# RIKEN-RCCS/EigenExa

Hardware: AMD Instinct MI355X
Metric: eigen_sx full-solve throughput (reference flop model: 4/3 N^3 + D&C GEMM + 2 nvec N^2) (higher is better)
Workload: dtype f64; 1 GPU; N=8192 random symmetric fp64 (counter-based R+R^T, seed 20240807), eigen_sx all eigenpairs, m_forward=64, m_backward=128; parallelism=1 GPU (1x1 grid)

## Files before the change

eigenexa_amd/_lib.py:

```python
import ctypes as C
import os

_HERE = os.path.dirname(os.path.abspath(__file__))
LIB_PATH = os.environ.get("EIGX_LIB") or os.path.join(_HERE, "lib", "libeigenexa_amd.so")

_c_double_p = C.POINTER(C.c_double)
_c_int_p = C.POINTER(C.c_int)

_INT, _PTR = C.c_int, C.c_void_p
_SOLVE = [_INT, _INT, _PTR, _INT, _PTR, _PTR, _INT, _INT, _INT, C.c_char]
_SOLVE_BC = [_INT, _INT, _INT, _PTR, _INT, _PTR, _PTR, _INT, _INT, _INT, _INT, C.c_char]
_RANGE = [_INT, _INT, _INT, _PTR, _INT, _PTR, _PTR, _INT, _INT, _INT, C.c_char]
_RANGE_V = [_INT, C.c_double, C.c_double, _INT, _c_int_p, _c_int_p, _PTR, _INT, _PTR, _PTR, _INT, _INT, _INT, C.c_char]
_GEV = [_INT, _PTR, _INT, _PTR, _INT, _PTR, _PTR, _INT]
_GEV_RANGE = [_INT, _INT, _INT, _PTR, _INT, _PTR, _INT, _PTR, _PTR, _INT, C.c_char]
_GEV_RANGE_V = [_INT, C.c_double, C.c_double, _INT, _c_int_p, _c_int_p, _PTR, _INT, _PTR, _INT, _PTR, _PTR, _INT, C.c_char]
_BATCH = [_INT, _INT, _PTR, _INT, C.c_int64, _PTR, _INT, _PTR, _INT, C.c_int64, C.c_char, _PTR]
_GEV_BATCH = [_INT, _INT, _PTR, _INT, C.c_int64, _PTR, _INT, C.c_int64, _PTR, _INT, _PTR, _INT, C.c_int64, C.c_char, _PTR]
_INDEX = [_INT, _INT, _INT]
_CHOL = [_INT, _PTR, _INT]
_TRSM = [C.c_char, _INT, _INT, _PTR, _INT, _PTR, _INT]
_REDUCE = [_INT, _PTR, _INT, _PTR, _INT]

SIGNATURES = {
# ... 132 lines not shown
}

HBATCH_RANGE_SIGNATURES = {
    "eigx_h_batch_range": (C.c_int, _BATCH_RANGE),
    "eigx_h_batch_range_dev": (C.c_int, _BATCH_RANGE),
}

LAB_SIGNATURES = {
    "eigx_dgemm_ex_dev": (C.c_int, [C.c_char, C.c_char, _INT, _INT, _INT, C.c_double, _PTR, _INT, _PTR, _INT, C.c_double, _PTR,
                                    _INT, _INT, _INT, _INT, _INT, _INT, _INT, C.c_int64, C.c_int64, C.c_int64, _INT, C.c_int64,
                                    C.c_int64, C.c_int64, _INT, _INT, _PTR, _PTR]),
    "eigx_dgemm_tri2_launch_tiles": (C.c_int, [_INT] * 8),
    "eigx_dgemm_gather_table_dev": (C.c_int, [_INT, _PTR, _PTR, _INT, _PTR, _INT, _PTR, _INT, _PTR, _PTR]),
}

_lib = None


def load():
    global _lib
    if _lib is not None:
        return _lib
    if not os.path.exists(LIB_PATH):
        raise RuntimeError(
            f"{LIB_PATH} not found: build it with tools/build_lib.sh (hipcc --offload-arch=gfx950). "
            "eigenexa_amd has no CPU fallback."
        )
    lib = C.CDLL(LIB_PATH, mode=C.RTLD_GLOBAL)
    for name, (res, args) in {**SIGNATURES, **GBATCH_SIGNATURES, **HGBATCH_SIGNATURES, **VBATCH_SIGNATURES,
                               **GVBATCH_SIGNATURES, **BATCH_RANGE_SIGNATURES, **HBATCH_RANGE_SIGNATURES}.items():
        fn = getattr(lib, name)
        fn.restype = res
        fn.argtypes = args
    for name, (res, args) in LAB_SIGNATURES.items():
        fn = getattr(lib, name, None)
        if fn is not None:
            fn.restype = res
            fn.argtypes = args
    _lib = lib
    return lib


def check(rc, what):
    if rc != 0:
        raise RuntimeError(f"{what} failed with code {rc}")
```

eigenexa_amd/csrc/api.hip:

```cpp
#include "eigx_context.h"
#include "eigx_comm.h"
#include "../../include/eigenexa_amd.h"
#include <cstring>

namespace eigx {
Context g_ctx;
}

using namespace eigx;

extern "C" {

int eigx_init(int device) {
  return eigx_init_multi(device, 0, 1, nullptr, 'C');
}

int eigx_get_device_count(void) {
  int ndev = 0;
  if (hipGetDeviceCount(&ndev) != hipSuccess) { (void)hipGetLastError(); return 0; }
  return ndev;
}

int eigx_get_rccl_unique_id(void* out128) {
  return comm_get_unique_id(out128);
// ... 313 lines not shown
  if (key == 6) return set_gemm_cstream(value);
  if (key == 7) return value > 0 ? set_reduce_knob(key, value) : -1;
  if (key == 8) return set_dc_chunk(value);
  if (key == 9) return comm_set_bounce(value);
  if (key == 15) return set_dc_pipe(value);
  if (key == 16) return set_dc_batch(value);
  if (key == 17 || key == 18 || key == 19) return set_range_knob(key, value);
  if (key == 20) return set_tri_nb(value);
  if (key == 21) return set_batch_nmax(value);
  if (key == 22) return set_hbatch_nmax(value);
  if (key == 23) return set_gbatch_nmax(value);
  if (key == 24) return set_hgbatch_nmax(value);
  if (key == 25) return set_gemm_latec_kmax(value);
  if (key == 26) return set_batch_range_route(value);
  if (key == 27) return set_batch_range_accept(value);
  return -1;
}

int eigx_dgemm_dev(char opa, char opb, int m, int n, int k, double alpha, const double* a, int lda,
                   const double* b, int ldb, double beta, double* c, int ldc, int tri_upper) {
  if (!g_ctx.initialized) return EIGX_ERR_NOT_INITIALIZED;
  EIGX_HIP_CHECK(hipStreamSynchronize(nullptr));
  dgemm_dev(g_ctx.stream, opa, opb, m, n, k, alpha, a, lda, b, ldb, beta, c, ldc, tri_upper ? 1 : 0,
            &g_ctx.grid);
  EIGX_HIP_CHECK(hipStreamSynchronize(g_ctx.stream));
  return EIGX_OK;
}

int eigx_dgemm_gather_dev(char opa, char opb, int m, int n, int k, double alpha, const double* a, int lda,
                          const double* b, int ldb, double beta, double* c, int ldc, const int* kmap_a,
// ... 11 lines not shown
```

eigenexa_amd/csrc/eigx_common.h:

```cpp
#pragma once
#include <hip/hip_runtime.h>
#include <cstdio>
#include <cstdlib>
#include <cstdint>
#include <cmath>
#include <vector>
#include <ctime>
#include <chrono>

#define EIGX_HIP_CHECK(expr)                                                        \
  do {                                                                              \
    hipError_t _e = (expr);                                                         \
    if (_e != hipSuccess) {                                                         \
      fprintf(stderr, "[eigx] HIP error %s at %s:%d: %s\n", hipGetErrorName(_e),    \
              __FILE__, __LINE__, hipGetErrorString(_e));                           \
      abort();                                                                      \
    }                                                                               \
  } while (0)

namespace eigx {

typedef double d4_t __attribute__((ext_vector_type(4)));

struct Grid {
// ... 42 lines not shown
};
inline char upper_case(char c) { return (c >= 'a' && c <= 'z') ? (char)(c - 'a' + 'A') : c; }
inline SolveRequest normalize_request(int n, int nvec, char mode) {
  mode = upper_case(mode);
  if (nvec == 0) mode = 'N';
  if (nvec < 0) nvec = -nvec;
  if (nvec > n) nvec = n;
  return SolveRequest{mode, nvec, mode != 'N'};
}


__global__ void fill_kernel(double* p, size_t n, double v);
__global__ void fill_vec_kernel(double* __restrict__ w, int n, double v);
__global__ void scale_vec_kernel(double* __restrict__ w, int n, double s);

void dgemm_dev(hipStream_t stream, char opA, char opB, int M, int N, int K, double alpha,
               const double* A, int lda, const double* B, int ldb, double beta, double* C, int ldc,
               int tri_mode = 0, const Grid* g = nullptr, const int* kmapA = nullptr,
               const int* cmapC = nullptr, int batch = 1, long strideA = 0, long strideB = 0, long strideC = 0,
               int batch2 = 1, long strideA2 = 0, long strideB2 = 0, long strideC2 = 0, int ownP = 1,
               int ownp = 0, const int* kmapB = nullptr, int tn_lo = 0, int tn_hi = 0x7fffffff);

int gemm_tri2_launch_tiles(int M, int N, const Grid& g, int tn_lo, int tn_hi);

struct GemmBatch {
  int M, N, K, pad;
  long offA, offB, offC;
  int offKA, offKB;
};
void dgemm_gather_batch_dev(hipStream_t stream, const GemmBatch* tab_dev, int nbatch, int maxM, int maxN,
                            const double* A, int lda, const double* B, int ldb, double* C, int ldc,
                            const int* kmapA, const int* kmapB);

inline void stage_trace(int rank, const char* what, long detail = -1) {
  static const bool on = getenv("EIGX_TRACE_STAGES") != nullptr;
  if (!on) return;
  timespec ts;
  clock_gettime(CLOCK_MONOTONIC, &ts);
  if (detail >= 0) fprintf(stderr, "[eigx stage] rank %d t=%.3f %s %ld\n", rank, ts.tv_sec % 100000 + ts.tv_nsec * 1e-9, what, detail);
  else fprintf(stderr, "[eigx stage] rank %d t=%.3f %s\n", rank, ts.tv_sec % 100000 + ts.tv_nsec * 1e-9, what);
  fflush(stderr);
}

int set_gemm_variant(int v);
int set_gemm_cstream(int v);
int set_gemm_latec_kmax(int v);
int set_bisect_threads(int v);
int set_bt_q(int v);
int set_reduce_knob(int key, int v);
int set_dc_chunk(int v);
int set_dc_pipe(int v);
int set_dc_batch(int v);
int set_batch_nmax(int v);
int set_hbatch_nmax(int v);
int get_batch_nmax();
int get_hbatch_nmax();
int set_gbatch_nmax(int v);
int set_hgbatch_nmax(int v);
int get_gbatch_nmax();
int set_batch_range_route(int v);
int set_batch_range_accept(int v);
int get_batch_range_route();
int get_batch_range_accept();
// ... 4 lines not shown
```

eigenexa_amd/csrc/gemm_f64.hip:

```cpp
#include "eigx_common.h"

namespace eigx {

namespace {

constexpr int BK = 16;
constexpr int LD_KC = BK + 1;
template <int WT> struct Geo {
  static constexpr int BM = 2 * WT, BN = 2 * WT;
  static constexpr int LD_MC = BM + 16;
  static constexpr int OPER = (BK * LD_MC > BM * LD_KC) ? BK * LD_MC : BM * LD_KC;
  static constexpr int NL = BM * BK / 256;
  static constexpr int NF = WT / 16;
};

struct GemmArgs {
  int M, N, K;
  double alpha, beta;
  const double* A;
  int lda;
  const double* B;
  int ldb;
  double* C;
  int ldc;
  int tri_mode;
  int Px, px, Py, py;
  const int* kmapA;
  const int* cmapC;
  const int* kmapB;
  long sA, sB, sC;
  long sA2, sB2, sC2;
  int ownP, ownp;
  int tri_gb;
  int tn_lo, tn_hi;
  int c_stream;
  int nrg, rg_h, rg_c1;
  unsigned rg_magic;
  const GemmBatch* btab;
};
__host__ __device__ inline int tri2_c0(const GemmArgs& g, int q, int tiles_n) {
  const long grow_min = (long)q * g.rg_h * 128 * g.Px + g.px;
  const unsigned x = grow_min > g.py ? (unsigned)(grow_min - g.py + g.Py - 1) : 0u;
#ifdef __HIP_DEVICE_COMPILE__
  const unsigned lc = (g.Py == 1) ? x : __umulhi(x, g.rg_magic);
#else
  const unsigned lc = (g.Py == 1) ? x : (unsigned)(((unsigned long long)x * g.rg_magic) >> 32);
#endif
  int c = (lc > (unsigned)(g.N - 1)) ? tiles_n : (int)(lc >> 7);
  if (c < g.tn_lo) c = g.tn_lo;
  if (c > g.rg_c1) c = g.rg_c1;
  return c;
}
typedef double d2s_t __attribute__((ext_vector_type(2)));

template <int WT>
__device__ __forceinline__ void load_map(int (&kc)[Geo<WT>::NL], const int* __restrict__ kmap, int k0, int Kmax,
                                         int tid) {
  constexpr int BM = Geo<WT>::BM, NL = Geo<WT>::NL;
  const int kb = k0 + tid / BM;
#pragma unroll
  for (int p = 0; p < NL; ++p) {
    const int k = kb + (256 / BM) * p;
    kc[p] = kmap[k < Kmax ? k : 0];
  }
}

template <bool KC, int WT, bool MAP>
__device__ __forceinline__ void load_slab(double (&r)[Geo<WT>::NL], const double* __restrict__ P, int ld, int m0,
                                          int k0, int Mmax, int Kmax, int tid, const int (&kc)[Geo<WT>::NL]) {
  constexpr int BM = Geo<WT>::BM, NL = Geo<WT>::NL;
  if (!KC) {
    const int m = m0 + (tid & (BM - 1));
    const int kb = k0 + tid / BM;
    const bool mok = m < Mmax;
    if (MAP) {
#pragma unroll
      for (int p = 0; p < NL; ++p) {
        const int k = kb + (256 / BM) * p;
        r[p] = (mok && k < Kmax) ? P[(size_t)m + (size_t)kc[p] * ld] : 0.0;
      }
    } else {
#pragma unroll
      for (int p = 0; p < NL; ++p) {
        const int k = kb + (256 / BM) * p;
        r[p] = (mok && k < Kmax) ? P[(size_t)m + (size_t)k * ld] : 0.0;
      }
    }
  } else {
    const int k = k0 + (tid & 15);
    const int mb = m0 + (tid >> 4);
    const bool kok = k < Kmax;
#pragma unroll
    for (int p = 0; p < NL; ++p) {
      const int m = mb + 16 * p;
      r[p] = (kok && m < Mmax) ? P[(size_t)k + (size_t)m * ld] : 0.0;
    }
  }
}

template <bool KC, int WT>
__device__ __forceinline__ void store_slab(const double (&r)[Geo<WT>::NL], double* __restrict__ S, int tid) {
  constexpr int BM = Geo<WT>::BM, NL = Geo<WT>::NL, LD_MC = Geo<WT>::LD_MC;
  if (!KC) {
    const int m = tid & (BM - 1);
    const int kb = tid / BM;
#pragma unroll
    for (int p = 0; p < NL; ++p) S[(kb + (256 / BM) * p) * LD_MC + m] = r[p];
  } else {
    const int k = tid & 15;
    const int mb = tid >> 4;
#pragma unroll
    for (int p = 0; p < NL; ++p) S[(mb + 16 * p) * LD_KC + k] = r[p];
  }
}

template <bool KC, int WT>
__device__ __forceinline__ double frag(const double* __restrict__ S, int m, int k) {
  return KC ? S[m * LD_KC + k] : S[k * Geo<WT>::LD_MC + m];
}

template <bool A_KC, bool B_KC, int WT, bool GATHER>
__global__ __launch_bounds__(256, 2) void gemm_f64_kernel(GemmArgs g) {
  extern __shared__ __attribute__((aligned(16))) double smem[];
  constexpr int BM = Geo<WT>::BM, BN = Geo<WT>::BN, OPER_DOUBLES = Geo<WT>::OPER, NL = Geo<WT>::NL, NF = Geo<WT>::NF;
  g.A += (long)blockIdx.y * g.sA + (long)blockIdx.z * g.sA2;
  g.B += (long)blockIdx.y * g.sB + (long)blockIdx.z * g.sB2;
  g.C += (long)blockIdx.y * g.sC + (long)blockIdx.z * g.sC2;
  if (g.btab) {
    const GemmBatch b = g.btab[blockIdx.y];
    g.M = b.M; g.N = b.N; g.K = b.K;
    g.A += b.offA; g.B += b.offB; g.C += b.offC;
    if (GATHER) { g.kmapA += b.offKA; g.kmapB += b.offKB; }
    if ((int)blockIdx.x >= ((g.M + BM - 1) / BM) * ((g.N + BN - 1) / BN)) return;
  }

  const int tid = threadIdx.x;
  const int lane = tid & 63;
// ... 42 lines not shown
          const int m = m0 + wm * WT + i * 16 + fm;
          acc[i][j][r] = (n < g.N && m < g.M) ? cscale * cp[m] : 0.0;
        }
      }
  } else {
#pragma unroll
    for (int j = 0; j < NF; ++j)
#pragma unroll
      for (int i = 0; i < NF; ++i) acc[i][j] = (d4_t){0.0, 0.0, 0.0, 0.0};
  }

  double ra[NL], rb[NL];
  int kca[NL], kcb[NL];
#pragma unroll
  for (int p = 0; p < NL; ++p) { kca[p] = 0; kcb[p] = 0; }
  const int nk = (g.K + BK - 1) / BK;
  if (GATHER) { load_map<WT>(kca, g.kmapA, 0, g.K, tid); load_map<WT>(kcb, g.kmapB, 0, g.K, tid); }
  load_slab<A_KC, WT, GATHER>(ra, g.A, g.lda, m0, 0, g.M, g.K, tid, kca);
  load_slab<B_KC, WT, GATHER>(rb, g.B, g.ldb, n0, 0, g.N, g.K, tid, kcb);
  if (GATHER && nk > 1) { load_map<WT>(kca, g.kmapA, BK, g.K, tid); load_map<WT>(kcb, g.kmapB, BK, g.K, tid); }
  store_slab<A_KC, WT>(ra, smem, tid);
  store_slab<B_KC, WT>(rb, smem + OPER_DOUBLES, tid);
  __syncthreads();

  for (int kt = 0; kt < nk; ++kt) {
    const int cur = kt & 1;
    if (kt + 1 < nk) {
      load_slab<A_KC, WT, GATHER>(ra, g.A, g.lda, m0, (kt + 1) * BK, g.M, g.K, tid, kca);
      load_slab<B_KC, WT, GATHER>(rb, g.B, g.ldb, n0, (kt + 1) * BK, g.N, g.K, tid, kcb);
      if (GATHER && kt + 2 < nk) {
        load_map<WT>(kca, g.kmapA, (kt + 2) * BK, g.K, tid);
        load_map<WT>(kcb, g.kmapB, (kt + 2) * BK, g.K, tid);
      }
    }
    const double* as = smem + cur * 2 * OPER_DOUBLES;
    const double* bs = as + OPER_DOUBLES;
#pragma unroll
    for (int ks = 0; ks < BK / 4; ++ks) {
      double fa[NF], fb[NF];
#pragma unroll
      for (int i = 0; i < NF; ++i) fa[i] = frag<A_KC, WT>(as, wm * WT + i * 16 + fm, ks * 4 + fk);
#pragma unroll
      for (int j = 0; j < NF; ++j) fb[j] = frag<B_KC, WT>(bs, wn * WT + j * 16 + fm, ks * 4 + fk);
#pragma unroll
// ... 75 lines not shown
  asm volatile("s_load_dword %0, %1, %2" : "=s"(v) : "s"(p), "s"(idx * 4) : "memory");
  return v;
}
template <bool MAP>
__device__ __forceinline__ void g2_cols(const int* __restrict__ kmap, int k0, int K, int wave, int& c0, int& c1) {
  const int k = k0 + 2 * wave;
  if (MAP) {
    c0 = 0; c1 = 0;
    if (k < K) c0 = g2_sload(kmap, k);
    if (k + 1 < K) c1 = g2_sload(kmap, k + 1);
  } else {
    c0 = k; c1 = k + 1;
  }
}

template <bool A_KC, bool B_KC, bool GATHER, bool LATE_C = false>
__global__ __launch_bounds__(256, 2) void gemm2_kernel(GemmArgs g) {
  static_assert(!LATE_C || (!A_KC && !B_KC && !GATHER), "late C: plain 'N','T' operands only");
  extern __shared__ __attribute__((aligned(16))) double smem[];
  constexpr int S = 4;
  constexpr int GI = 4;
  constexpr int CI = 8;
  g.A += (long)blockIdx.y * g.sA + (long)blockIdx.z * g.sA2;
  g.B += (long)blockIdx.y * g.sB + (long)blockIdx.z * g.sB2;
  g.C += (long)blockIdx.y * g.sC + (long)blockIdx.z * g.sC2;

  const int tid = threadIdx.x;
  const int lane = tid & 63;
  const int wave = __builtin_amdgcn_readfirstlane(tid >> 6);
  const int wm = wave & 1, wn = wave >> 1;

  const int tiles_m = (g.M + 127) / 128;
  const int tiles_n = (g.N + 127) / 128;
// ... 43 lines not shown
    const int rows = (tiles_m - rg * 8 < 8) ? tiles_m - rg * 8 : 8;
    tn = rem / rows;
    tm = rg * 8 + rem - tn * rows;
  }
  const int m0 = tm * 128, n0 = tn * 128;
  if (g.tri_mode != 0) {
    if (g.ownP > 1 && (tn % g.ownP) != g.ownp) return;
    if (tn < g.tn_lo || tn >= g.tn_hi) return;
    const long grow_min = (long)m0 * g.Px + g.px;
    const int jmax = (n0 + 127 < g.N - 1) ? n0 + 127 : g.N - 1;
    const long gcol_max = (long)jmax * g.Py + g.py;
    if (grow_min > gcol_max) return;
  }

  const int fm = lane & 15, fk = lane >> 4;
  const int nk = (g.K + G2_BK - 1) / G2_BK;

  auto ncol = [&](int j, int rho) { return B_KC ? j * 16 + rho : (j >> 1) * 32 + 2 * rho + (j & 1); };

  d4_t acc[4][4];
  const bool use_c = !LATE_C && (g.beta != 0.0) && (g.alpha != 0.0);
  if (use_c) {
    const double cscale = g.beta / g.alpha;
#pragma unroll
    for (int j = 0; j < 4; ++j)
#pragma unroll
      for (int r = 0; r < 4; ++r) {
        const int n = n0 + wn * 64 + ncol(j, fk + 4 * r);
        const double* cp = g.C + (size_t)n * g.ldc;
        if (!A_KC) {
// ... 245 lines not shown
  g.Px = grid.Px; g.px = grid.px; g.Py = grid.Py; g.py = grid.py;
  return tri2_plan(g);
}

int set_gemm_variant(int v) { const int old = g_gemm_variant; g_gemm_variant = v; return old; }
int set_gemm_cstream(int v) { const int old = g_gemm_cstream; g_gemm_cstream = v; return old; }
int set_gemm_latec_kmax(int v) {
  if (v < 0 || v >= 512) return -1;
  const int old = g_gemm_latec_kmax; g_gemm_latec_kmax = v; return old;
}

void dgemm_dev(hipStream_t stream, char opA, char opB, int M, int N, int K, double alpha, const double* A,
               int lda, const double* B, int ldb, double beta, double* C, int ldc, int tri_mode,
               const Grid* grid, const int* kmapA, const int* cmapC, int batch, long strideA, long strideB,
               long strideC, int batch2, long strideA2, long strideB2, long strideC2, int ownP, int ownp,
               const int* kmapB, int tn_lo, int tn_hi) {
  if (M <= 0 || N <= 0 || batch <= 0 || batch2 <= 0) return;
  if (alpha == 0.0) K = 0;
  GemmArgs g;
  g.M = M; g.N = N; g.K = K; g.alpha = alpha; g.beta = beta;
  g.A = A; g.lda = lda; g.B = B; g.ldb = ldb; g.C = C; g.ldc = ldc;
  g.tri_mode = tri_mode;
  g.kmapA = (opA == 'N' || opA == 'n') ? kmapA : nullptr;
  g.cmapC = cmapC;
  g.kmapB = (opB == 'T' || opB == 't') ? kmapB : nullptr;
  g.sA = strideA; g.sB = strideB; g.sC = strideC;
  g.sA2 = strideA2; g.sB2 = strideB2; g.sC2 = strideC2;
  g.ownP = ownP; g.ownp = ownp; g.tri_gb = 1;
  g.tn_lo = tn_lo; g.tn_hi = tn_hi;
  g.nrg = 0; g.rg_h = 8; g.rg_c1 = 0; g.rg_magic = 0; g.btab = nullptr;
  g.c_stream = (tri_mode != 0 && g_gemm_cstream) ? 1 : 0;
  g.Px = grid ? grid->Px : 1; g.px = grid ? grid->px : 0;
  g.Py = grid ? grid->Py : 1; g.py = grid ? grid->py : 0;
  const bool a_kc = (opA == 'T' || opA == 't');
  const bool b_kc = (opB == 'N' || opB == 'n');
  const bool gather = g.kmapA || g.kmapB;
  if ((!gather || (g.kmapA && g.kmapB && !a_kc && !b_kc)) && gemm2_ok(g, a_kc, b_kc, batch, batch2)) {
    const long t128 = (long)ceil_div(M, 128) * ceil_div(N, 128) * batch * batch2;
    if (tri_mode != 0 || t128 >= 192 || g_gemm_variant == 3) {
      int gx2 = ceil_div(M, 128) * ceil_div(N, 128);
      if (tri_mode == 1) {
        const int t = ceil_div(N > M ? N : M, 128);
        g.tri_gb = (t >= 96) ? 8 : (t >= 24 ? 4 : (t >= 8 ? 2 : 1));
        const int nb = ceil_div(t, g.tri_gb);
        const int nblk = nb * (nb + 1) / 2;
        gx2 = 8 * ceil_div(nblk, 8) * g.tri_gb * g.tri_gb;
      }
      if (tri_mode == 2 && batch == 1 && batch2 == 1 && ownP == 1) {
        const int total = tri2_plan(g);
        if (total == 0) return;
        gx2 = total;
      }
      dim3 grd2(gx2, batch, batch2), blk2(256);
      const size_t shmem2 = (size_t)4 * G2_STAGE * sizeof(double);
#define EIGX_LAUNCH2(AK, BK_, GA_, LC_)                                                            \
  do {                                                                                             \
    static bool attr_set2 = false;                                                                 \
    if (!attr_set2) {                                                                              \
      EIGX_HIP_CHECK(hipFuncSetAttribute((const void*)gemm2_kernel<AK, BK_, GA_, LC_>,             \
                                         hipFuncAttributeMaxDynamicSharedMemorySize, (int)shmem2)); \
      attr_set2 = true;                                                                            \
    }                                                                                              \
    hipLaunchKernelGGL((gemm2_kernel<AK, BK_, GA_, LC_>), grd2, blk2, shmem2, stream, g);          \
  } while (0)
      const bool late_c = tri_mode == 1 && beta != 0.0 && K <= g_gemm_latec_kmax && !g.c_stream;
      if (gather) EIGX_LAUNCH2(false, false, true, false);
      else if (a_kc && b_kc) EIGX_LAUNCH2(true, true, false, false);
      else if (a_kc) EIGX_LAUNCH2(true, false, false, false);
      else if (b_kc) EIGX_LAUNCH2(false, true, false, false);
      else if (late_c) EIGX_LAUNCH2(false, false, false, true);
      else EIGX_LAUNCH2(false, false, false, false);
#undef EIGX_LAUNCH2
      EIGX_HIP_CHECK(hipGetLastError());
      return;
    }
  }
  const long tiles128 = (long)ceil_div(M, 128) * ceil_div(N, 128) * batch * batch2;
  const bool small = (tri_mode == 0) && tiles128 < 192;
  const int bm = small ? 64 : 128;
  const int tiles = ceil_div(M, bm) * ceil_div(N, bm);
  dim3 grd(tiles, batch, batch2), blk(256);
#define EIGX_LAUNCH(AK, BK_, WT_, GA_)                                                             \
  do {                                                                                             \
    const size_t shmem = (size_t)4 * Geo<WT_>::OPER * sizeof(double);                              \
    static bool attr_set = false;                                                                  \
    if (!attr_set) {                                                                               \
      EIGX_HIP_CHECK(hipFuncSetAttribute((const void*)gemm_f64_kernel<AK, BK_, WT_, GA_>,          \
                                         hipFuncAttributeMaxDynamicSharedMemorySize, (int)shmem)); \
      attr_set = true;                                                                             \
    }                                                                                              \
    hipLaunchKernelGGL((gemm_f64_kernel<AK, BK_, WT_, GA_>), grd, blk, shmem, stream, g);          \
  } while (0)
#define EIGX_LAUNCH_T(AK, BK_) do { if (small) EIGX_LAUNCH(AK, BK_, 32, false); else EIGX_LAUNCH(AK, BK_, 64, false); } while (0)
  if (g.kmapA || g.kmapB) {
    if (a_kc || b_kc || !g.kmapA || !g.kmapB) {
      fprintf(stderr, "[eigx] dgemm gather needs opA='N', opB='T' and both maps\n");
      abort();
    }
    if (small) EIGX_LAUNCH(false, false, 32, true); else EIGX_LAUNCH(false, false, 64, true);
  } else if (a_kc && b_kc) EIGX_LAUNCH_T(true, true);
  else if (a_kc && !b_kc) EIGX_LAUNCH_T(true, false);
  else if (!a_kc && b_kc) EIGX_LAUNCH_T(false, true);
  else EIGX_LAUNCH_T(false, false);
#undef EIGX_LAUNCH_T
#undef EIGX_LAUNCH
  EIGX_HIP_CHECK(hipGetLastError());
}

void dgemm_gather_batch_dev(hipStream_t stream, const GemmBatch* tab_dev, int nbatch, int maxM, int maxN,
                            const double* A, int lda, const double* B, int ldb, double* C, int ldc,
                            const int* kmapA, const int* kmapB) {
  if (nbatch <= 0 || maxM <= 0 || maxN <= 0) return;
  GemmArgs g;
  g.M = maxM; g.N = maxN; g.K = 0; g.alpha = 1.0; g.beta = 0.0;
  g.A = A; g.lda = lda; g.B = B; g.ldb = ldb; g.C = C; g.ldc = ldc;
  g.tri_mode = 0; g.kmapA = kmapA; g.cmapC = nullptr; g.kmapB = kmapB;
  g.sA = g.sB = g.sC = 0; g.sA2 = g.sB2 = g.sC2 = 0;
  g.ownP = 1; g.ownp = 0; g.tri_gb = 1; g.tn_lo = 0; g.tn_hi = 0x7fffffff;
  g.nrg = 0; g.rg_h = 8; g.rg_c1 = 0; g.rg_magic = 0; g.c_stream = 0;
  g.Px = 1; g.px = 0; g.Py = 1; g.py = 0;
  g.btab = tab_dev;
  constexpr int WT = 32;
  const int tiles = ceil_div(maxM, Geo<WT>::BM) * ceil_div(maxN, Geo<WT>::BN);
  const size_t shmem = (size_t)4 * Geo<WT>::OPER * sizeof(double);
  static bool attr_set = false;
  if (!attr_set) {
    EIGX_HIP_CHECK(hipFuncSetAttribute((const void*)gemm_f64_kernel<false, false, WT, true>,
                                       hipFuncAttributeMaxDynamicSharedMemorySize, (int)shmem));
    attr_set = true;
  }
  hipLaunchKernelGGL((gemm_f64_kernel<false, false, WT, true>), dim3(tiles, nbatch, 1), dim3(256), shmem, stream, g);
  EIGX_HIP_CHECK(hipGetLastError());
}

// ... 2 lines not shown
```

eigenexa_amd/csrc/gemm_lab.hip:

```cpp
#include "eigx_context.h"
#include "../../include/eigenexa_amd.h"
#include "../../include/eigenexa_amd_gemm_lab.h"
#include <climits>

using namespace eigx;

extern "C" {

int eigx_dgemm_ex_dev(char opa, char opb, int m, int n, int k, double alpha, const double* a, int lda, const double* b,
                      int ldb, double beta, double* c, int ldc, int tri_mode, int px_n, int px, int py_n, int py, int batch,
                      int64_t stride_a, int64_t stride_b, int64_t stride_c, int batch2, int64_t stride_a2, int64_t stride_b2,
                      int64_t stride_c2, int tn_lo, int tn_hi, const int* kmap_a, const int* kmap_b) {
  if (!g_ctx.initialized) return EIGX_ERR_NOT_INITIALIZED;
  if (tri_mode < 0 || tri_mode > 2) return EIGX_ERR_BAD_ARG;
  if (px_n < 1 || py_n < 1 || px < 0 || px >= px_n || py < 0 || py >= py_n) return EIGX_ERR_BAD_ARG;
  if (kmap_a || kmap_b) {
    const bool nt = (opa == 'N' || opa == 'n') && (opb == 'T' || opb == 't');
    if (!nt || !kmap_a || !kmap_b) return EIGX_ERR_BAD_ARG;
  }
  Grid grid;
  grid.Px = px_n; grid.px = px; grid.Py = py_n; grid.py = py;
  grid.nranks = px_n * py_n;
  EIGX_HIP_CHECK(hipStreamSynchronize(nullptr));
  dgemm_dev(g_ctx.stream, opa, opb, m, n, k, alpha, a, lda, b, ldb, beta, c, ldc, tri_mode, &grid, kmap_a, nullptr, batch,
            (long)stride_a, (long)stride_b, (long)stride_c, batch2, (long)stride_a2, (long)stride_b2, (long)stride_c2, 1, 0,
            kmap_b, tn_lo, tn_hi);
  EIGX_HIP_CHECK(hipStreamSynchronize(g_ctx.stream));
  return EIGX_OK;
}

int eigx_dgemm_tri2_launch_tiles(int m, int n, int px_n, int px, int py_n, int py, int tn_lo, int tn_hi) {
  if (px_n < 1 || py_n < 1 || px < 0 || px >= px_n || py < 0 || py >= py_n) return EIGX_ERR_BAD_ARG;
  Grid grid;
  grid.Px = px_n; grid.px = px; grid.Py = py_n; grid.py = py;
  return gemm_tri2_launch_tiles(m, n, grid, tn_lo, tn_hi);
}

int eigx_dgemm_gather_table_dev(int nbatch, const int64_t* entries, const double* a, int lda, const double* b, int ldb,
                                double* c, int ldc, const int* kmap_a, const int* kmap_b) {
  if (!g_ctx.initialized) return EIGX_ERR_NOT_INITIALIZED;
  if (nbatch < 0 || (nbatch > 0 && (!entries || !kmap_a || !kmap_b))) return EIGX_ERR_BAD_ARG;
  if (nbatch == 0) return EIGX_OK;
  std::vector<GemmBatch> tab(nbatch);
// ... 24 lines not shown
```

eigenexa_amd/csrc/trbak.hip:

```cpp
#include "eigx_context.h"
#include "eigx_comm.h"
#include "../../include/eigenexa_amd.h"

namespace eigx {

namespace {

constexpr int GCH = 512;
int g_bt_q = 0;

__global__ void zero_below_kernel(double* __restrict__ A, int lda, int n, int band, int rows_pad) {
  const int j = blockIdx.y;
  const int len = j - band + 1;
  double* col = A + (size_t)j * lda;
  const int lo = len > 0 ? len : 0;
  const int hi = rows_pad < lda ? rows_pad : lda;
  for (int r = lo + blockIdx.x * blockDim.x + threadIdx.x; r < hi; r += gridDim.x * blockDim.x) col[r] = 0.0;
}

__device__ __forceinline__ int tri_idx(int r, int c) { return r * (r + 1) / 2 + c; }

__global__ __launch_bounds__(256) void tbuild_kernel(const double* __restrict__ Gall, int maxchunks, int gch, int mb,
                                                     int mbe, int nsub, int n, const double* __restrict__ A, int lda,
                                                     const double* __restrict__ e, int lde, int band,
// ... 104 lines not shown
  if (q > 1) {
    double* Gs = ctx.pool.get_t<double>("bt.Gs", (size_t)nblk * msz);
    double* Y = ctx.pool.get_t<double>("bt.Y", (size_t)nblk * msz);
    hipLaunchKernelGGL(gsum_kernel, dim3(64, nblk), dim3(256), 0, st, Gall, maxchunks, mbe, Gs);
    for (int h = mb; h < mbe; h *= 2) {
      const int np = mbe / (2 * h);
      const long dstep = (long)2 * h * (mbe + 1);
      dgemm_dev(st, 'N', 'N', h, h, h, 1.0, Gs + h, mbe, Tall, mbe, 0.0, Y, h, 0, nullptr, nullptr, nullptr, np, dstep,
                dstep, (long)h * h, nblk, (long)msz, (long)msz, (long)np * h * h);
      dgemm_dev(st, 'N', 'N', h, h, h, -1.0, Tall + (size_t)h * (mbe + 1), mbe, Y, h, 0.0, Tall + h, mbe, 0, nullptr,
                nullptr, nullptr, np, dstep, (long)h * h, dstep, nblk, (long)msz, (long)np * h * h, (long)msz);
    }
  }
}

static void bt_apply_range(Context& ctx, int nvec, const double* V, int ldv, double* Z, int ldz, int band, int jstart,
                           int jend, int mb, int q) {
  if (jend <= jstart) return;
  hipStream_t st = ctx.stream;
  const BtRange g = bt_range_geom(ctx, band, jstart, jend, mb, q);
  const int mbe = g.mbe;
  double* W = ctx.pool.get_t<double>("bt.W", (size_t)(mbe > 512 ? mbe : 512) * nvec);
  double* X = ctx.pool.get_t<double>("bt.X", (size_t)(mbe > 512 ? mbe : 512) * nvec);
  for (int b = 0; b < g.nblk; ++b) {
    const int j0 = jstart + b * mbe;
    const int mbk = (jend - j0 < mbe) ? jend - j0 : mbe;
    const int rows = j0 + mbk - band;
    const double* Vb = V + (size_t)j0 * ldv;
    const double* T = g.Tall + (size_t)b * g.msz;
    dgemm_dev(st, 'T', 'N', mbk, nvec, rows, 1.0, Vb, ldv, Z, ldz, 0.0, W, mbe);
    dgemm_dev(st, 'N', 'N', mbk, nvec, mbk, 1.0, T, mbe, W, mbe, 0.0, X, mbe);
    dgemm_dev(st, 'N', 'N', rows, nvec, mbk, -1.0, Vb, ldv, X, mbe, 1.0, Z, ldz);
  }
}

struct BtPlan { int mb, q, mbe, js, rows_pad; };
static BtPlan bt_plan(int n, int mb, int band) {
  BtPlan p;
  if (mb < 8) mb = 8;
  if (mb > 128) mb = 128;
  int q = 1;
  if (mb == 128 && n >= 2048) q = (n >= 6144) ? 4 : 2;
  if (g_bt_q > 0 && mb == 128) q = g_bt_q;
  p.mb = mb; p.q = q; p.mbe = mb * q;
  const int total = n - band;
  const int nsup = (q > 1) ? total / p.mbe : 0;
  p.js = (nsup > 0) ? n - nsup * p.mbe : n;
// ... 107 lines not shown
    const BtRange g = bt_range_geom(ctx, band, j0, j1, p.mb, q);
    int rows_pad = g.maxchunks * g.gch;
    if (rows_pad > ldv) rows_pad = ldv;
    hipLaunchKernelGGL(unpack_refl_kernel, dim3(ceil_div(rows_pad, 256) < 64 ? ceil_div(rows_pad, 256) : 64, j1 - j0), dim3(256),
                       0, st, (const double*)recv->local, cnt, nxc, j0, j1, band, rows_pad, G.Px, G.Py, G.row_major, Vg, ldv);
    double* Vs = Vg - (size_t)j0 * ldv;
    bt_prepare_range(ctx, st, n, Vs, ldv, e, lde, band, j0, j1, p.mb, q);
    if (nvec > 0) bt_apply_range(ctx, nvec, Vs, ldv, Z, ldz, band, j0, j1, p.mb, q);
  };
  for (int j0 = band; j0 < p.js; j0 += plain_cols) run_group(j0, (j0 + plain_cols < p.js) ? j0 + plain_cols : p.js, 1);
  for (int j0 = p.js; j0 < n; j0 += group_cols) run_group(j0, (j0 + group_cols < n) ? j0 + group_cols : n, p.q);
  EIGX_HIP_CHECK(hipGetLastError());
}

int set_bt_q(int v) { const int old = g_bt_q; g_bt_q = v; return old; }

}
```

Before: 19470 GFLOP/s.

## Skip structurally zero K ranges in back-transform GEMMs via per-tile K windows

Adds a per-row-tile K window to the f64 GEMM kernels, letting each 128-row tile clamp its reduction range to where the operand is nonzero. The back-transform's three GEMMs pass windows that follow the trapezoidal/triangular shape of the reflector block V and the triangular T, so tiles skip K slabs that are known to be zero. This is meant to cut wasted FLOPs and memory traffic in the Householder back-transformation. The cost is extra kernel template instantiations and a correctness dependence on the assumed zero structure of V and T.

```diff
diff --git a/eigenexa_amd/_lib.py b/eigenexa_amd/_lib.py
--- a/eigenexa_amd/_lib.py
+++ b/eigenexa_amd/_lib.py
@@ -170,6 +170,10 @@
     "eigx_dgemm_gather_table_dev": (C.c_int, [_INT, _PTR, _PTR, _INT, _PTR, _INT, _PTR, _INT, _PTR, _PTR]),
 }
 
+KWIN_LAB_SIGNATURES = {
+    "eigx_dgemm_kwin_dev": (C.c_int, LAB_SIGNATURES["eigx_dgemm_ex_dev"][1] + [_INT, _INT]),
+}
+
 _lib = None
 
 
@@ -188,7 +192,7 @@
         fn = getattr(lib, name)
         fn.restype = res
         fn.argtypes = args
-    for name, (res, args) in LAB_SIGNATURES.items():
+    for name, (res, args) in {**LAB_SIGNATURES, **KWIN_LAB_SIGNATURES}.items():
         fn = getattr(lib, name, None)
         if fn is not None:
             fn.restype = res
diff --git a/eigenexa_amd/csrc/api.hip b/eigenexa_amd/csrc/api.hip
--- a/eigenexa_amd/csrc/api.hip
+++ b/eigenexa_amd/csrc/api.hip
@@ -351,6 +351,7 @@
   if (key == 25) return set_gemm_latec_kmax(value);
   if (key == 26) return set_batch_range_route(value);
   if (key == 27) return set_batch_range_accept(value);
+  if (key == 28) return set_bt_kwin(value);
   return -1;
 }
 
diff --git a/eigenexa_amd/csrc/eigx_common.h b/eigenexa_amd/csrc/eigx_common.h
--- a/eigenexa_amd/csrc/eigx_common.h
+++ b/eigenexa_amd/csrc/eigx_common.h
@@ -3,6 +3,7 @@
 #include <cstdio>
 #include <cstdlib>
 #include <cstdint>
+#include <climits>
 #include <cmath>
 #include <vector>
 #include <ctime>
@@ -80,12 +81,14 @@
 __global__ void fill_vec_kernel(double* __restrict__ w, int n, double v);
 __global__ void scale_vec_kernel(double* __restrict__ w, int n, double s);
 
+constexpr int KWIN_LO_NONE = INT_MIN, KWIN_HI_NONE = INT_MAX;
 void dgemm_dev(hipStream_t stream, char opA, char opB, int M, int N, int K, double alpha,
                const double* A, int lda, const double* B, int ldb, double beta, double* C, int ldc,
                int tri_mode = 0, const Grid* g = nullptr, const int* kmapA = nullptr,
                const int* cmapC = nullptr, int batch = 1, long strideA = 0, long strideB = 0, long strideC = 0,
                int batch2 = 1, long strideA2 = 0, long strideB2 = 0, long strideC2 = 0, int ownP = 1,
-               int ownp = 0, const int* kmapB = nullptr, int tn_lo = 0, int tn_hi = 0x7fffffff);
+               int ownp = 0, const int* kmapB = nullptr, int tn_lo = 0, int tn_hi = 0x7fffffff,
+               int klo0 = KWIN_LO_NONE, int khi0 = KWIN_HI_NONE);
 
 int gemm_tri2_launch_tiles(int M, int N, const Grid& g, int tn_lo, int tn_hi);
 
@@ -113,6 +116,7 @@
 int set_gemm_latec_kmax(int v);
 int set_bisect_threads(int v);
 int set_bt_q(int v);
+int set_bt_kwin(int v);
 int set_reduce_knob(int key, int v);
 int set_dc_chunk(int v);
 int set_dc_pipe(int v);
diff --git a/eigenexa_amd/csrc/gemm_f64.hip b/eigenexa_amd/csrc/gemm_f64.hip
--- a/eigenexa_amd/csrc/gemm_f64.hip
+++ b/eigenexa_amd/csrc/gemm_f64.hip
@@ -37,7 +37,15 @@
   int nrg, rg_h, rg_c1;
   unsigned rg_magic;
   const GemmBatch* btab;
+  int klo0, khi0;
 };
+__device__ __forceinline__ void k_window(const GemmArgs& g, int m0, int& klo, int& khi) {
+  const long mw = m0 & ~127;
+  const long lo = mw + g.klo0, hi = mw + g.khi0;
+  klo = lo > 0 ? (int)(lo < g.K ? lo : g.K) : 0;
+  khi = hi < g.K ? (int)(hi > 0 ? hi : 0) : g.K;
+  if (khi <= klo) { klo = 0; khi = 0; }
+}
 __host__ __device__ inline int tri2_c0(const GemmArgs& g, int q, int tiles_n) {
   const long grow_min = (long)q * g.rg_h * 128 * g.Px + g.px;
   const unsigned x = grow_min > g.py ? (unsigned)(grow_min - g.py + g.Py - 1) : 0u;
@@ -65,9 +73,10 @@
   }
 }
 
-template <bool KC, int WT, bool MAP>
+template <bool KC, int WT, bool MAP, bool WIN = false>
 __device__ __forceinline__ void load_slab(double (&r)[Geo<WT>::NL], const double* __restrict__ P, int ld, int m0,
-                                          int k0, int Mmax, int Kmax, int tid, const int (&kc)[Geo<WT>::NL]) {
+                                          int k0, int Mmax, int Kmax, int tid, const int (&kc)[Geo<WT>::NL],
+                                          int Kmin = 0) {
   constexpr int BM = Geo<WT>::BM, NL = Geo<WT>::NL;
   if (!KC) {
     const int m = m0 + (tid & (BM - 1));
@@ -83,13 +92,13 @@
 #pragma unroll
       for (int p = 0; p < NL; ++p) {
         const int k = kb + (256 / BM) * p;
-        r[p] = (mok && k < Kmax) ? P[(size_t)m + (size_t)k * ld] : 0.0;
+        r[p] = (mok && k < Kmax && (!WIN || k >= Kmin)) ? P[(size_t)m + (size_t)k * ld] : 0.0;
       }
     }
   } else {
     const int k = k0 + (tid & 15);
     const int mb = m0 + (tid >> 4);
-    const bool kok = k < Kmax;
+    const bool kok = k < Kmax && (!WIN || k >= Kmin);
 #pragma unroll
     for (int p = 0; p < NL; ++p) {
       const int m = mb + 16 * p;
@@ -119,8 +128,9 @@
   return KC ? S[m * LD_KC + k] : S[k * Geo<WT>::LD_MC + m];
 }
 
-template <bool A_KC, bool B_KC, int WT, bool GATHER>
+template <bool A_KC, bool B_KC, int WT, bool GATHER, bool WIN = false>
 __global__ __launch_bounds__(256, 2) void gemm_f64_kernel(GemmArgs g) {
+  static_assert(!(WIN && GATHER), "no K window with gather maps");
   extern __shared__ __attribute__((aligned(16))) double smem[];
   constexpr int BM = Geo<WT>::BM, BN = Geo<WT>::BN, OPER_DOUBLES = Geo<WT>::OPER, NL = Geo<WT>::NL, NF = Geo<WT>::NF;
   g.A += (long)blockIdx.y * g.sA + (long)blockIdx.z * g.sA2;
@@ -193,20 +203,23 @@
   int kca[NL], kcb[NL];
 #pragma unroll
   for (int p = 0; p < NL; ++p) { kca[p] = 0; kcb[p] = 0; }
-  const int nk = (g.K + BK - 1) / BK;
+  int klo = 0, khi = g.K;
+  if (WIN) k_window(g, m0, klo, khi);
+  const int kt0 = WIN ? klo / BK : 0;
+  const int nk = (khi + BK - 1) / BK;
   if (GATHER) { load_map<WT>(kca, g.kmapA, 0, g.K, tid); load_map<WT>(kcb, g.kmapB, 0, g.K, tid); }
-  load_slab<A_KC, WT, GATHER>(ra, g.A, g.lda, m0, 0, g.M, g.K, tid, kca);
-  load_slab<B_KC, WT, GATHER>(rb, g.B, g.ldb, n0, 0, g.N, g.K, tid, kcb);
+  load_slab<A_KC, WT, GATHER, WIN>(ra, g.A, g.lda, m0, kt0 * BK, g.M, khi, tid, kca, klo);
+  load_slab<B_KC, WT, GATHER, WIN>(rb, g.B, g.ldb, n0, kt0 * BK, g.N, khi, tid, kcb, klo);
   if (GATHER && nk > 1) { load_map<WT>(kca, g.kmapA, BK, g.K, tid); load_map<WT>(kcb, g.kmapB, BK, g.K, tid); }
   store_slab<A_KC, WT>(ra, smem, tid);
   store_slab<B_KC, WT>(rb, smem + OPER_DOUBLES, tid);
   __syncthreads();
 
-  for (int kt = 0; kt < nk; ++kt) {
-    const int cur = kt & 1;
+  for (int kt = kt0; kt < nk; ++kt) {
+    const int cur = (kt - kt0) & 1;
     if (kt + 1 < nk) {
-      load_slab<A_KC, WT, GATHER>(ra, g.A, g.lda, m0, (kt + 1) * BK, g.M, g.K, tid, kca);
-      load_slab<B_KC, WT, GATHER>(rb, g.B, g.ldb, n0, (kt + 1) * BK, g.N, g.K, tid, kcb);
+      load_slab<A_KC, WT, GATHER, WIN>(ra, g.A, g.lda, m0, (kt + 1) * BK, g.M, khi, tid, kca, klo);
+      load_slab<B_KC, WT, GATHER, WIN>(rb, g.B, g.ldb, n0, (kt + 1) * BK, g.N, khi, tid, kcb, klo);
       if (GATHER && kt + 2 < nk) {
         load_map<WT>(kca, g.kmapA, (kt + 2) * BK, g.K, tid);
         load_map<WT>(kcb, g.kmapB, (kt + 2) * BK, g.K, tid);
@@ -312,9 +325,10 @@
   }
 }
 
-template <bool A_KC, bool B_KC, bool GATHER, bool LATE_C = false>
+template <bool A_KC, bool B_KC, bool GATHER, bool LATE_C = false, bool WIN = false>
 __global__ __launch_bounds__(256, 2) void gemm2_kernel(GemmArgs g) {
   static_assert(!LATE_C || (!A_KC && !B_KC && !GATHER), "late C: plain 'N','T' operands only");
+  static_assert(!WIN || (!GATHER && !LATE_C), "K window: no gather maps, early C only");
   extern __shared__ __attribute__((aligned(16))) double smem[];
   constexpr int S = 4;
   constexpr int GI = 4;
@@ -388,6 +402,14 @@
   }
 
   const int fm = lane & 15, fk = lane >> 4;
+  if (WIN) {
+    int klo, khi;
+    k_window(g, m0, klo, khi);
+    const int kb = klo & ~(G2_BK - 1);
+    g.A += A_KC ? (long)kb : (long)kb * g.lda;
+    g.B += B_KC ? (long)kb : (long)kb * g.ldb;
+    g.K = khi - kb;
+  }
   const int nk = (g.K + G2_BK - 1) / G2_BK;
 
   auto ncol = [&](int j, int rho) { return B_KC ? j * 16 + rho : (j >> 1) * 32 + 2 * rho + (j & 1); };
@@ -663,8 +685,13 @@
                int lda, const double* B, int ldb, double beta, double* C, int ldc, int tri_mode,
                const Grid* grid, const int* kmapA, const int* cmapC, int batch, long strideA, long strideB,
                long strideC, int batch2, long strideA2, long strideB2, long strideC2, int ownP, int ownp,
-               const int* kmapB, int tn_lo, int tn_hi) {
+               const int* kmapB, int tn_lo, int tn_hi, int klo0, int khi0) {
   if (M <= 0 || N <= 0 || batch <= 0 || batch2 <= 0) return;
+  const bool win = klo0 != KWIN_LO_NONE || khi0 != KWIN_HI_NONE;
+  if (win && (tri_mode != 0 || kmapA || kmapB)) {
+    fprintf(stderr, "[eigx] dgemm: a K window goes with neither a tri mode nor gather maps\n");
+    abort();
+  }
   if (alpha == 0.0) K = 0;
   GemmArgs g;
   g.M = M; g.N = N; g.K = K; g.alpha = alpha; g.beta = beta;
@@ -679,6 +706,7 @@
   g.tn_lo = tn_lo; g.tn_hi = tn_hi;
   g.nrg = 0; g.rg_h = 8; g.rg_c1 = 0; g.rg_magic = 0; g.btab = nullptr;
   g.c_stream = (tri_mode != 0 && g_gemm_cstream) ? 1 : 0;
+  g.klo0 = klo0; g.khi0 = khi0;
   g.Px = grid ? grid->Px : 1; g.px = grid ? grid->px : 0;
   g.Py = grid ? grid->Py : 1; g.py = grid ? grid->py : 0;
   const bool a_kc = (opA == 'T' || opA == 't');
@@ -702,23 +730,29 @@
       }
       dim3 grd2(gx2, batch, batch2), blk2(256);
       const size_t shmem2 = (size_t)4 * G2_STAGE * sizeof(double);
-#define EIGX_LAUNCH2(AK, BK_, GA_, LC_)                                                            \
+#define EIGX_LAUNCH2(AK, BK_, GA_, LC_, WN_)                                                       \
   do {                                                                                             \
     static bool attr_set2 = false;                                                                 \
     if (!attr_set2) {                                                                              \
-      EIGX_HIP_CHECK(hipFuncSetAttribute((const void*)gemm2_kernel<AK, BK_, GA_, LC_>,             \
+      EIGX_HIP_CHECK(hipFuncSetAttribute((const void*)gemm2_kernel<AK, BK_, GA_, LC_, WN_>,        \
                                          hipFuncAttributeMaxDynamicSharedMemorySize, (int)shmem2)); \
       attr_set2 = true;                                                                            \
     }                                                                                              \
-    hipLaunchKernelGGL((gemm2_kernel<AK, BK_, GA_, LC_>), grd2, blk2, shmem2, stream, g);          \
+    hipLaunchKernelGGL((gemm2_kernel<AK, BK_, GA_, LC_, WN_>), grd2, blk2, shmem2, stream, g);     \
   } while (0)
       const bool late_c = tri_mode == 1 && beta != 0.0 && K <= g_gemm_latec_kmax && !g.c_stream;
-      if (gather) EIGX_LAUNCH2(false, false, true, false);
-      else if (a_kc && b_kc) EIGX_LAUNCH2(true, true, false, false);
-      else if (a_kc) EIGX_LAUNCH2(true, false, false, false);
-      else if (b_kc) EIGX_LAUNCH2(false, true, false, false);
-      else if (late_c) EIGX_LAUNCH2(false, false, false, true);
-      else EIGX_LAUNCH2(false, false, false, false);
+      if (win) {
+        if (a_kc && b_kc) EIGX_LAUNCH2(true, true, false, false, true);
+        else if (a_kc) EIGX_LAUNCH2(true, false, false, false, true);
+        else if (b_kc) EIGX_LAUNCH2(false, true, false, false, true);
+        else EIGX_LAUNCH2(false, false, false, false, true);
+      }
+      else if (gather) EIGX_LAUNCH2(false, false, true, false, false);
+      else if (a_kc && b_kc) EIGX_LAUNCH2(true, true, false, false, false);
+      else if (a_kc) EIGX_LAUNCH2(true, false, false, false, false);
+      else if (b_kc) EIGX_LAUNCH2(false, true, false, false, false);
+      else if (late_c) EIGX_LAUNCH2(false, false, false, true, false);
+      else EIGX_LAUNCH2(false, false, false, false, false);
 #undef EIGX_LAUNCH2
       EIGX_HIP_CHECK(hipGetLastError());
       return;
@@ -729,29 +763,31 @@
   const int bm = small ? 64 : 128;
   const int tiles = ceil_div(M, bm) * ceil_div(N, bm);
   dim3 grd(tiles, batch, batch2), blk(256);
-#define EIGX_LAUNCH(AK, BK_, WT_, GA_)                                                             \
+#define EIGX_LAUNCH(AK, BK_, WT_, GA_, WN_)                                                        \
   do {                                                                                             \
     const size_t shmem = (size_t)4 * Geo<WT_>::OPER * sizeof(double);                              \
     static bool attr_set = false;                                                                  \
     if (!attr_set) {                                                                               \
-      EIGX_HIP_CHECK(hipFuncSetAttribute((const void*)gemm_f64_kernel<AK, BK_, WT_, GA_>,          \
+      EIGX_HIP_CHECK(hipFuncSetAttribute((const void*)gemm_f64_kernel<AK, BK_, WT_, GA_, WN_>,     \
                                          hipFuncAttributeMaxDynamicSharedMemorySize, (int)shmem)); \
       attr_set = true;                                                                             \
     }                                                                                              \
-    hipLaunchKernelGGL((gemm_f64_kernel<AK, BK_, WT_, GA_>), grd, blk, shmem, stream, g);          \
+    hipLaunchKernelGGL((gemm_f64_kernel<AK, BK_, WT_, GA_, WN_>), grd, blk, shmem, stream, g);     \
   } while (0)
-#define EIGX_LAUNCH_T(AK, BK_) do { if (small) EIGX_LAUNCH(AK, BK_, 32, false); else EIGX_LAUNCH(AK, BK_, 64, false); } while (0)
+#define EIGX_LAUNCH_W(AK, BK_, WN_) do { if (small) EIGX_LAUNCH(AK, BK_, 32, false, WN_); else EIGX_LAUNCH(AK, BK_, 64, false, WN_); } while (0)
+#define EIGX_LAUNCH_T(AK, BK_) do { if (win) EIGX_LAUNCH_W(AK, BK_, true); else EIGX_LAUNCH_W(AK, BK_, false); } while (0)
   if (g.kmapA || g.kmapB) {
     if (a_kc || b_kc || !g.kmapA || !g.kmapB) {
       fprintf(stderr, "[eigx] dgemm gather needs opA='N', opB='T' and both maps\n");
       abort();
     }
-    if (small) EIGX_LAUNCH(false, false, 32, true); else EIGX_LAUNCH(false, false, 64, true);
+    if (small) EIGX_LAUNCH(false, false, 32, true, false); else EIGX_LAUNCH(false, false, 64, true, false);
   } else if (a_kc && b_kc) EIGX_LAUNCH_T(true, true);
   else if (a_kc && !b_kc) EIGX_LAUNCH_T(true, false);
   else if (!a_kc && b_kc) EIGX_LAUNCH_T(false, true);
   else EIGX_LAUNCH_T(false, false);
 #undef EIGX_LAUNCH_T
+#undef EIGX_LAUNCH_W
 #undef EIGX_LAUNCH
   EIGX_HIP_CHECK(hipGetLastError());
 }
@@ -767,6 +803,7 @@
   g.sA = g.sB = g.sC = 0; g.sA2 = g.sB2 = g.sC2 = 0;
   g.ownP = 1; g.ownp = 0; g.tri_gb = 1; g.tn_lo = 0; g.tn_hi = 0x7fffffff;
   g.nrg = 0; g.rg_h = 8; g.rg_c1 = 0; g.rg_magic = 0; g.c_stream = 0;
+  g.klo0 = KWIN_LO_NONE; g.khi0 = KWIN_HI_NONE;
   g.Px = 1; g.px = 0; g.Py = 1; g.py = 0;
   g.btab = tab_dev;
   constexpr int WT = 32;
diff --git a/eigenexa_amd/csrc/gemm_lab.hip b/eigenexa_amd/csrc/gemm_lab.hip
--- a/eigenexa_amd/csrc/gemm_lab.hip
+++ b/eigenexa_amd/csrc/gemm_lab.hip
@@ -1,16 +1,17 @@
 #include "eigx_context.h"
 #include "../../include/eigenexa_amd.h"
 #include "../../include/eigenexa_amd_gemm_lab.h"
+#include "../../include/eigenexa_amd_kwin_lab.h"
 #include <climits>
 
 using namespace eigx;
 
 extern "C" {
 
-int eigx_dgemm_ex_dev(char opa, char opb, int m, int n, int k, double alpha, const double* a, int lda, const double* b,
-                      int ldb, double beta, double* c, int ldc, int tri_mode, int px_n, int px, int py_n, int py, int batch,
-                      int64_t stride_a, int64_t stride_b, int64_t stride_c, int batch2, int64_t stride_a2, int64_t stride_b2,
-                      int64_t stride_c2, int tn_lo, int tn_hi, const int* kmap_a, const int* kmap_b) {
+static int dgemm_lab(char opa, char opb, int m, int n, int k, double alpha, const double* a, int lda, const double* b,
+                     int ldb, double beta, double* c, int ldc, int tri_mode, int px_n, int px, int py_n, int py, int batch,
+                     int64_t stride_a, int64_t stride_b, int64_t stride_c, int batch2, int64_t stride_a2, int64_t stride_b2,
+                     int64_t stride_c2, int tn_lo, int tn_hi, const int* kmap_a, const int* kmap_b, int klo0, int khi0) {
   if (!g_ctx.initialized) return EIGX_ERR_NOT_INITIALIZED;
   if (tri_mode < 0 || tri_mode > 2) return EIGX_ERR_BAD_ARG;
   if (px_n < 1 || py_n < 1 || px < 0 || px >= px_n || py < 0 || py >= py_n) return EIGX_ERR_BAD_ARG;
@@ -18,15 +19,33 @@
     const bool nt = (opa == 'N' || opa == 'n') && (opb == 'T' || opb == 't');
     if (!nt || !kmap_a || !kmap_b) return EIGX_ERR_BAD_ARG;
   }
+  if ((klo0 != KWIN_LO_NONE || khi0 != KWIN_HI_NONE) && (tri_mode != 0 || kmap_a || kmap_b)) return EIGX_ERR_BAD_ARG;
   Grid grid;
   grid.Px = px_n; grid.px = px; grid.Py = py_n; grid.py = py;
   grid.nranks = px_n * py_n;
   EIGX_HIP_CHECK(hipStreamSynchronize(nullptr));
   dgemm_dev(g_ctx.stream, opa, opb, m, n, k, alpha, a, lda, b, ldb, beta, c, ldc, tri_mode, &grid, kmap_a, nullptr, batch,
             (long)stride_a, (long)stride_b, (long)stride_c, batch2, (long)stride_a2, (long)stride_b2, (long)stride_c2, 1, 0,
-            kmap_b, tn_lo, tn_hi);
+            kmap_b, tn_lo, tn_hi, klo0, khi0);
   EIGX_HIP_CHECK(hipStreamSynchronize(g_ctx.stream));
   return EIGX_OK;
+}
+
+int eigx_dgemm_ex_dev(char opa, char opb, int m, int n, int k, double alpha, const double* a, int lda, const double* b,
+                      int ldb, double beta, double* c, int ldc, int tri_mode, int px_n, int px, int py_n, int py, int batch,
+                      int64_t stride_a, int64_t stride_b, int64_t stride_c, int batch2, int64_t stride_a2, int64_t stride_b2,
+                      int64_t stride_c2, int tn_lo, int tn_hi, const int* kmap_a, const int* kmap_b) {
+  return dgemm_lab(opa, opb, m, n, k, alpha, a, lda, b, ldb, beta, c, ldc, tri_mode, px_n, px, py_n, py, batch, stride_a,
+                   stride_b, stride_c, batch2, stride_a2, stride_b2, stride_c2, tn_lo, tn_hi, kmap_a, kmap_b, KWIN_LO_NONE,
+                   KWIN_HI_NONE);
+}
+
+int eigx_dgemm_kwin_dev(char opa, char opb, int m, int n, int k, double alpha, const double* a, int lda, const double* b,
+                        int ldb, double beta, double* c, int ldc, int tri_mode, int px_n, int px, int py_n, int py, int batch,
+                        int64_t stride_a, int64_t stride_b, int64_t stride_c, int batch2, int64_t stride_a2, int64_t stride_b2,
+                        int64_t stride_c2, int tn_lo, int tn_hi, const int* kmap_a, const int* kmap_b, int klo0, int khi0) {
+  return dgemm_lab(opa, opb, m, n, k, alpha, a, lda, b, ldb, beta, c, ldc, tri_mode, px_n, px, py_n, py, batch, stride_a,
+                   stride_b, stride_c, batch2, stride_a2, stride_b2, stride_c2, tn_lo, tn_hi, kmap_a, kmap_b, klo0, khi0);
 }
 
 int eigx_dgemm_tri2_launch_tiles(int m, int n, int px_n, int px, int py_n, int py, int tn_lo, int tn_hi) {
diff --git a/eigenexa_amd/csrc/trbak.hip b/eigenexa_amd/csrc/trbak.hip
--- a/eigenexa_amd/csrc/trbak.hip
+++ b/eigenexa_amd/csrc/trbak.hip
@@ -8,6 +8,7 @@
 
 constexpr int GCH = 512;
 int g_bt_q = 0;
+int g_bt_kwin = 1;
 
 __global__ void zero_below_kernel(double* __restrict__ A, int lda, int n, int band, int rows_pad) {
   const int j = blockIdx.y;
@@ -142,6 +143,13 @@
   }
 }
 
+static void gemm_kwin(hipStream_t st, char opA, int M, int N, int K, double alpha, const double* A, int lda, const double* B,
+                      int ldb, double beta, double* C, int ldc, int klo0, int khi0) {
+  if (!g_bt_kwin) { klo0 = KWIN_LO_NONE; khi0 = KWIN_HI_NONE; }
+  dgemm_dev(st, opA, 'N', M, N, K, alpha, A, lda, B, ldb, beta, C, ldc, 0, nullptr, nullptr, nullptr, 1, 0, 0, 0, 1, 0, 0, 0, 1,
+            0, nullptr, 0, 0x7fffffff, klo0, khi0);
+}
+
 static void bt_apply_range(Context& ctx, int nvec, const double* V, int ldv, double* Z, int ldz, int band, int jstart,
                            int jend, int mb, int q) {
   if (jend <= jstart) return;
@@ -156,9 +164,9 @@
     const int rows = j0 + mbk - band;
     const double* Vb = V + (size_t)j0 * ldv;
     const double* T = g.Tall + (size_t)b * g.msz;
-    dgemm_dev(st, 'T', 'N', mbk, nvec, rows, 1.0, Vb, ldv, Z, ldz, 0.0, W, mbe);
-    dgemm_dev(st, 'N', 'N', mbk, nvec, mbk, 1.0, T, mbe, W, mbe, 0.0, X, mbe);
-    dgemm_dev(st, 'N', 'N', rows, nvec, mbk, -1.0, Vb, ldv, X, mbe, 1.0, Z, ldz);
+    gemm_kwin(st, 'T', mbk, nvec, rows, 1.0, Vb, ldv, Z, ldz, 0.0, W, mbe, KWIN_LO_NONE, j0 - band + 128);
+    gemm_kwin(st, 'N', mbk, nvec, mbk, 1.0, T, mbe, W, mbe, 0.0, X, mbe, KWIN_LO_NONE, 128);
+    gemm_kwin(st, 'N', rows, nvec, mbk, -1.0, Vb, ldv, X, mbe, 1.0, Z, ldz, band - j0, KWIN_HI_NONE);
   }
 }
 
@@ -296,5 +304,6 @@
 }
 
 int set_bt_q(int v) { const int old = g_bt_q; g_bt_q = v; return old; }
-
-}
+int set_bt_kwin(int v) { const int old = g_bt_kwin; g_bt_kwin = v ? 1 : 0; return old; }
+
+}
diff --git a/include/eigenexa_amd_kwin_lab.h b/include/eigenexa_amd_kwin_lab.h
--- /dev/null
+++ b/include/eigenexa_amd_kwin_lab.h
@@ -0,0 +1,19 @@
+#ifndef EIGENEXA_AMD_KWIN_LAB_H
+#define EIGENEXA_AMD_KWIN_LAB_H
+
+#include <stdint.h>
+
+#ifdef __cplusplus
+extern "C" {
+#endif
+
+int eigx_dgemm_kwin_dev(char opa, char opb, int m, int n, int k, double alpha, const double* a_dev, int lda, const double* b_dev,
+                        int ldb, double beta, double* c_dev, int ldc, int tri_mode, int px_n, int px, int py_n, int py, int batch,
+                        int64_t stride_a, int64_t stride_b, int64_t stride_c, int batch2, int64_t stride_a2, int64_t stride_b2,
+                        int64_t stride_c2, int tn_lo, int tn_hi, const int* kmap_a_dev, const int* kmap_b_dev, int klo0,
+                        int khi0);
+
+#ifdef __cplusplus
+}
+#endif
+#endif
```

Measured after the change: 19490 GFLOP/s (median of 2 runs). About the same (+0.1%).
